# Amos-Chen98/neo-planner

Hardware: AMD Instinct MI355X
Metric: trajectories/sec (batched replan) (higher is better)
Workload: dtype f32x; 1 GPU; cfg2: 40 x 4096 trajectories x 20 waypoints per step per GPU, 1 x 300^3 f32 ESDF per GPU (trilinear, pillars + 80 canopy boxes), each optimised to L-BFGS-B termination; batch_per_launch=4096, pieces=21, dims=3, esdf_voxels=27000000, layout=brick, parallelism=scene-sharded x1, launches_in_flight_per_gpu=4

## Files before the change

neo-planner_amd/csrc/neo_device.hpp:

```cpp
#pragma once
#include <type_traits>
#include <hip/hip_runtime.h>
#include <hip/hip_fp16.h>

#include "../../include/neo_planner.h"
#include "neo_wave.hpp"

namespace neo {

constexpr int kSlots = 4;

struct DevParams {
  double v_max, T_min, T_max, safe_dis, delta_t;
  double w[4];
  double coll_tol;
  double ftol, gtol;
  int maxls, maxiter, maxfun, stale_T;
  int dbg;
  struct F32 {
    float T_min, T_span;
    float dt, inv_dt;
    float vmax2, safe;
    float w[4];
  } f;
// ... 103 lines not shown
  }
};

template <typename E>
__device__ __forceinline__ float elem_to_float(E v);
template <>
__device__ __forceinline__ float elem_to_float<float>(float v) { return v; }
template <>
__device__ __forceinline__ float elem_to_float<__half>(__half v) { return __half2float(v); }

typedef unsigned long long u64_align4 __attribute__((aligned(4)));
typedef unsigned int u32_align2 __attribute__((aligned(2)));
template <typename E>
__device__ __forceinline__ void load_pair(const E *p, float &a, float &b);
template <>
__device__ __forceinline__ void load_pair<float>(const float *p, float &a, float &b) {
  const unsigned long long u = *reinterpret_cast<const u64_align4 *>(p);
  a = __uint_as_float((unsigned int)(u & 0xffffffffull));
  b = __uint_as_float((unsigned int)(u >> 32));
}
__device__ __forceinline__ void buffer_load_pair_f32(__amdgpu_buffer_rsrc_t rsrc, unsigned int off, unsigned int soff,
                                                     float &a, float &b) {
  const auto v = __builtin_amdgcn_raw_buffer_load_b64(rsrc, (int)off, (int)soff, 0);
  a = __uint_as_float(v[0]);
  b = __uint_as_float(v[1]);
}
template <>
__device__ __forceinline__ void load_pair<__half>(const __half *p, float &a, float &b) {
  const unsigned int u = *reinterpret_cast<const u32_align2 *>(p);
  a = __half2float(__ushort_as_half((unsigned short)(u & 0xffffu)));
  b = __half2float(__ushort_as_half((unsigned short)(u >> 16)));
}

template <typename Real, typename E, int LAYOUT>
struct Lookup3D {
  const Map3D &m;
  __amdgpu_buffer_rsrc_t rsrc;
  float inv, off[3], hi[3];
  __device__ __forceinline__ explicit Lookup3D(const Map3D &m_)
      : m(m_), rsrc(__builtin_amdgcn_make_buffer_rsrc(const_cast<void *>(m_.data), 0, (int)m_.bytes, 0x00020000)) {
    inv = m_.f_inv;
#pragma unroll
    for (int k = 0; k < 3; ++k) {
      off[k] = m_.f_off[k];
      hi[k] = m_.f_hi[k];
    }
  }
  struct Addr {
    int i0[3];
    Real fr[3];
    bool inside;
  };
  struct Raw {
    float c[2][2][2];
  };
  static constexpr bool gather_ahead = sizeof(E) == 4;
  static __device__ __forceinline__ void pin(Raw &q) {
#pragma unroll
    for (int k = 0; k < 8; ++k) q.c[k >> 2][(k >> 1) & 1][k & 1] = opaque(q.c[k >> 2][(k >> 1) & 1][k & 1]);
  }

  template <int D>
  __device__ __forceinline__ Addr prepare(const Real (&pos)[D], bool on = true) const {
#pragma clang fp contract(on)
    static_assert(D == 3, "the 3-D map needs D = 3");
    const int n[3] = {m.nx, m.ny, m.nz};
    const double org[3] = {m.ox, m.oy, m.oz};
    Addr a;
    a.inside = on;
    if constexpr (sizeof(Real) == 4) {
#pragma unroll
      for (int k = 0; k < 3; ++k) {
        const float um = fmaf(pos[k], inv, off[k]);
        if (!(um >= -0.5f && um < hi[k])) a.inside = false;
        const int i = min(max((int)floorf(um), 0), n[k] - 2);
        a.i0[k] = i;
        a.fr[k] = __builtin_amdgcn_fmed3f(um - (float)i, 0.0f, 1.0f);
      }
      if (!a.inside) a.i0[0] = a.i0[1] = a.i0[2] = 0;
      return a;
    }
#pragma unroll
    for (int k = 0; k < 3; ++k) {
      Real u = (Real)(((double)pos[k] - org[k]) * m.d_inv);
      if (!(u >= Real(0) && u < (Real)n[k])) a.inside = false;
      u -= Real(0.5);
      const int i = min(max((int)floor(u), 0), n[k] - 2);
      a.i0[k] = i;
      a.fr[k] = fmin(fmax(u - (Real)i, Real(0)), Real(1));
    }
    if (!a.inside) a.i0[0] = a.i0[1] = a.i0[2] = 0;
    return a;
  }
  __device__ __forceinline__ Raw load(const Addr &a) const {
    const E *vox = static_cast<const E *>(m.data);
    Raw q;
    if (LAYOUT == 2 || (LAYOUT == 9 && m.layout == NEO_LAYOUT_CELL8)) {
      const unsigned int cell = __umul24(__umul24((unsigned)a.i0[2], (unsigned)m.ny) + (unsigned)a.i0[1], (unsigned)m.nx) +
                                (unsigned)a.i0[0];
      if constexpr (sizeof(E) == 4) {
        const auto lo = __builtin_amdgcn_raw_buffer_load_b128(rsrc, (int)(cell * 32u), 0, 0);
        const auto hi = __builtin_amdgcn_raw_buffer_load_b128(rsrc, (int)(cell * 32u + 16u), 0, 0);
        q.c[0][0][0] = __uint_as_float(lo[0]); q.c[0][0][1] = __uint_as_float(lo[1]);
        q.c[0][1][0] = __uint_as_float(lo[2]); q.c[0][1][1] = __uint_as_float(lo[3]);
        q.c[1][0][0] = __uint_as_float(hi[0]); q.c[1][0][1] = __uint_as_float(hi[1]);
        q.c[1][1][0] = __uint_as_float(hi[2]); q.c[1][1][1] = __uint_as_float(hi[3]);
      } else {
        const auto v = __builtin_amdgcn_raw_buffer_load_b128(rsrc, (int)(cell * 16u), 0, 0);
#pragma unroll
        for (int w = 0; w < 4; ++w) {
          q.c[w >> 1][w & 1][0] = __half2float(__ushort_as_half((unsigned short)(v[w] & 0xffffu)));
          q.c[w >> 1][w & 1][1] = __half2float(__ushort_as_half((unsigned short)(v[w] >> 16)));
        }
      }
    } else if (LAYOUT == 3 || (LAYOUT == 9 && m.layout == NEO_LAYOUT_BRICK)) {
      constexpr int SHX = sizeof(E) == 4 ? 1 : 2, CX = (1 << SHX) + 1;
      const unsigned int bx = (unsigned)a.i0[0] >> SHX, by = (unsigned)a.i0[1] >> 1, bz = (unsigned)a.i0[2] >> 1;
      const unsigned int lx = (unsigned)a.i0[0] & ((1u << SHX) - 1u), ly = (unsigned)a.i0[1] & 1u, lz = (unsigned)a.i0[2] & 1u;
      const unsigned int blk = __umul24(__umul24(bz, (unsigned)m.nby) + by, (unsigned)m.nbx) + bx;
      const unsigned int in_line = (lz * 3u + ly) * (unsigned)CX + lx;
#pragma unroll
      for (int dz = 0; dz < 2; ++dz)
#pragma unroll
        for (int dy = 0; dy < 2; ++dy) {
          const unsigned int so = (unsigned)((dz * 3 + dy) * CX);
          if constexpr (sizeof(E) == 4) {
            const auto v = __builtin_amdgcn_raw_buffer_load_b64(rsrc, (int)(blk * 128u + in_line * 4u + so * 4u), 0, 0);
            q.c[dz][dy][0] = __uint_as_float(v[0]);
            q.c[dz][dy][1] = __uint_as_float(v[1]);
          } else {
            load_pair<E>(vox + blk * 64u + in_line + so, q.c[dz][dy][0], q.c[dz][dy][1]);
          }
        }
    } else if (LAYOUT == 0 || (LAYOUT == 9 && m.layout == NEO_LAYOUT_LINEAR)) {
      const unsigned int base = __umul24(__umul24((unsigned)a.i0[2], (unsigned)m.ny) + (unsigned)a.i0[1], (unsigned)m.nx) +
                                (unsigned)a.i0[0];
      const unsigned int sy = (unsigned)m.nx, sz = (unsigned)m.nx * (unsigned)m.ny;
#pragma unroll
      for (int dz = 0; dz < 2; ++dz)
#pragma unroll
        for (int dy = 0; dy < 2; ++dy) {
          const unsigned int so = (dy ? sy : 0u) + (dz ? sz : 0u);
          if constexpr (sizeof(E) == 4)
            buffer_load_pair_f32(rsrc, base * 4u, so * 4u, q.c[dz][dy][0], q.c[dz][dy][1]);
          else
            load_pair<E>(vox + base + so, q.c[dz][dy][0], q.c[dz][dy][1]);
        }
    } else {
      const unsigned int cell = __umul24(__umul24((unsigned)a.i0[2], (unsigned)m.ny) + (unsigned)a.i0[1], (unsigned)m.nx) +
                                (unsigned)a.i0[0];
      if constexpr (sizeof(E) == 4) {
        const auto lo = __builtin_amdgcn_raw_buffer_load_b128(rsrc, (int)(cell * 16u), 0, 0);
        const auto hi = __builtin_amdgcn_raw_buffer_load_b128(rsrc, (int)(cell * 16u + 16u), 0, 0);
        q.c[0][0][0] = __uint_as_float(lo[0]); q.c[0][1][0] = __uint_as_float(lo[1]);
        q.c[1][0][0] = __uint_as_float(lo[2]); q.c[1][1][0] = __uint_as_float(lo[3]);
        q.c[0][0][1] = __uint_as_float(hi[0]); q.c[0][1][1] = __uint_as_float(hi[1]);
        q.c[1][0][1] = __uint_as_float(hi[2]); q.c[1][1][1] = __uint_as_float(hi[3]);
      } else {
        const auto v = __builtin_amdgcn_raw_buffer_load_b128(rsrc, (int)(cell * 8u), 0, 0);
#pragma unroll
        for (int dx = 0; dx < 2; ++dx)
#pragma unroll
          for (int dz = 0; dz < 2; ++dz) {
            const unsigned int u = v[2 * dx + dz];
            q.c[dz][0][dx] = __half2float(__ushort_as_half((unsigned short)(u & 0xffffu)));
            q.c[dz][1][dx] = __half2float(__ushort_as_half((unsigned short)(u >> 16)));
          }
      }
    }
    return q;
  }
  template <int D>
  __device__ __forceinline__ Real finish(const Addr &a, const Raw &q, Real (&g)[D]) const {
#pragma clang fp contract(on)
#pragma unroll
    for (int d = 0; d < D; ++d) g[d] = Real(0);
    if (!a.inside) return Real(10000);
    const Real fx = a.fr[0], fy = a.fr[1], fz = a.fr[2];
    const Real inv_res = sizeof(Real) == 4 ? (Real)m.f_inv : (Real)m.d_inv;
    const Real c000 = (Real)q.c[0][0][0], c100 = (Real)q.c[0][0][1], c010 = (Real)q.c[0][1][0], c110 = (Real)q.c[0][1][1];
    const Real c001 = (Real)q.c[1][0][0], c101 = (Real)q.c[1][0][1], c011 = (Real)q.c[1][1][0], c111 = (Real)q.c[1][1][1];
    const Real dx00 = c100 - c000, dx10 = c110 - c010, dx01 = c101 - c001, dx11 = c111 - c011;
    const Real c00 = c000 + fx * dx00, c10 = c010 + fx * dx10;
    const Real c01 = c001 + fx * dx01, c11 = c011 + fx * dx11;
    const Real c0 = c00 + fy * (c10 - c00), c1 = c01 + fy * (c11 - c01);
    const Real dx0 = dx00 + fy * (dx10 - dx00), dx1 = dx01 + fy * (dx11 - dx01);
    const Real dy0 = c10 - c00, dy1 = c11 - c01;
    g[0] = (dx0 + fz * (dx1 - dx0)) * inv_res;
    g[1] = (dy0 + fz * (dy1 - dy0)) * inv_res;
    g[2] = (c1 - c0) * inv_res;
    return c0 + fz * (c1 - c0);
  }
  template <int D>
  __device__ __forceinline__ Real fetch(const Real (&pos)[D], Real (&g)[D], bool &inside) const {
    const Addr a = prepare<D>(pos);
    inside = a.inside;
    return finish<D>(a, load(a), g);
  }
};

__host__ __device__ __forceinline__ int sample_lanes_per_piece_fwd(int M);

struct WaveLanes {
  static constexpr int W = kWave;
  static constexpr int S = 1;
  static constexpr int dl(int D) { return D; }
  static __device__ __forceinline__ int lane() { return lane_id(); }
  static __device__ __forceinline__ int piece() { return lane_id(); }
  static __device__ __forceinline__ int dim0() { return 0; }
  static __device__ __forceinline__ int base() { return 0; }
  template <class T> static __device__ __forceinline__ T sum_dims(T v) { return v; }
  template <class T> static __device__ __forceinline__ T read(T v, int src ) { return rdlane(v, src); }
  template <class T> static __device__ __forceinline__ T prev(T v, T fill) { return from_prev(v, fill); }
  template <class T> static __device__ __forceinline__ T next(T v, T fill) { return from_next(v, fill); }
  template <class T> static __device__ __forceinline__ T sum(T v) { return wave_sum(v); }
  static __device__ __forceinline__ int any(int pred) { return __any(pred); }
  static __host__ __device__ __forceinline__ int lanes_per_piece(int M);
};

template <int W_>
struct GroupLanes {
  static_assert(W_ == 16 || W_ == 8, "a group is a DPP row or half of one");
  static constexpr int W = W_;
  static constexpr int S = 1;
  static constexpr int dl(int D) { return D; }
  static __device__ __forceinline__ int piece() { return lane_id() & (W - 1); }
  static __device__ __forceinline__ int dim0() { return 0; }
  static __device__ __forceinline__ int lane() { return lane_id() & (W - 1); }
  static __device__ __forceinline__ int base() { return lane_id() & ~(W - 1); }
  template <class T> static __device__ __forceinline__ T sum_dims(T v) { return v; }
  template <class T, class Op>
  static __device__ __forceinline__ T reduce(T v, Op op) {
    if constexpr (W == 16) {
      return __shfl(row_scan(v, op), base() + W - 1, kWave);
    } else {
      v = op(v, dpp<0xB1>(v)); v = op(v, dpp<0x4E>(v)); v = op(v, dpp<0x141>(v));
      return v;
    }
  }
  template <class T> static __device__ __forceinline__ T sum(T v) { return reduce(v, OpAdd()); }
  template <class T> static __device__ __forceinline__ T max_nonneg(T v) { return reduce(v, OpMax()); }
  static __device__ __forceinline__ int any(int pred) {
    return reduce(pred ? 1 : 0, [](int a, int b) { return a | b; });
  }
  template <class T>
  static __device__ __forceinline__ T read(T v, int src ) {
    return __shfl(v, base() + src, kWave);
  }
  template <class T> static __device__ __forceinline__ T prev(T v, T fill) {
    const T o = dpp<0x138>(v);
    return lane() == 0 ? fill : o;
  }
  template <class T> static __device__ __forceinline__ T next(T v, T fill) {
    const T o = dpp<0x130>(v);
    return lane() == W - 1 ? fill : o;
  }
  static __host__ __device__ __forceinline__ int lanes_per_piece(int M) {
    int L = W / M;
    if (L < 1) L = 1;
    if (L >= 8) L = (L >= 16 && W >= 16) ? 16 : 8;
    return L;
  }
};

template <int D_>
struct WaveLanesPD {
  static constexpr int W = kWave;
  static constexpr int S = D_;
  static constexpr int dl(int) { return 1; }
  static __device__ __forceinline__ int lane() { return lane_id(); }
  static __device__ __forceinline__ int base() { return 0; }
  static __device__ __forceinline__ int piece() { return (lane_id() * ((65536 + S - 1) / S)) >> 16; }
  static __device__ __forceinline__ int dim0() { return lane_id() - S * piece(); }
  template <class T> static __device__ __forceinline__ T read(T v, int q ) { return rdlane(v, S * q); }
  template <class T> static __device__ __forceinline__ T prev(T v, T fill) {
#pragma unroll
    for (int k = 0; k < S; ++k) v = dpp<0x138>(v);
    return lane_lt(S) ? fill : v;
  }
  template <class T> static __device__ __forceinline__ T next(T v, T fill) {
#pragma unroll
    for (int k = 0; k < S; ++k) v = dpp<0x130>(v);
    return lane_ge(kWave - S) ? fill : v;
  }
  template <class T> static __device__ __forceinline__ T sum(T v) { return wave_sum(v); }
  static __device__ __forceinline__ int any(int pred) { return __any(pred); }
  template <class T> static __device__ __forceinline__ T sum_dims(T v) {
    T acc = v, t = v;
#pragma unroll
    for (int k = 1; k < S; ++k) {
      t = dpp<0x130>(t);
      acc += t;
    }
    return acc;
  }
  static __host__ __device__ __forceinline__ int lanes_per_piece(int M) { return sample_lanes_per_piece_fwd(M); }
};

struct PlanDynamic {
  static constexpr bool dynamic = true;
  static constexpr bool fold_acc = false, fold_rows = false, pcr_mult = false, pcr_xch = false, sl_cache = false,
                        trace = false, coeff_out = false;
  static constexpr bool gather_ahead = false;
};
struct PlanFixedX {
  static constexpr bool dynamic = false;
  static constexpr bool fold_acc = true, fold_rows = true, pcr_mult = true, pcr_xch = true, sl_cache = true,
                        trace = false, coeff_out = false;
  static constexpr bool gather_ahead = true;
};
template <class Plan, bool K>
__host__ __device__ __forceinline__ constexpr bool plan_pick(bool run_time) {
  if constexpr (Plan::dynamic)
    return run_time;
  else
    return K;
}

template <int D, int DL = D, typename Num = double>
struct Traj {
  int M, n, nq, L;
  Num T, tau;
  Num i1, i2, i3, i4;
  Num P0[DL], P1[DL];
  Num V0[DL], A0[DL], V1[DL], A1[DL];
  Num c[6][DL];
  int ns;
  Num N[2][2];
  const double *head, *tail;
  const Num *bnd;
  Num *pcr_xch = nullptr;
  Num *pcr_mult = nullptr;
};

template <int D, class LG, bool TAIL, int DL, typename Num>
__device__ __forceinline__ Num bstate(const Traj<D, DL, Num> &t, int k, int dl) {
  if constexpr (LG::S == 1 && LG::W == kWave)
    return (Num)(TAIL ? t.tail : t.head)[k * D + dl];
  else
    return t.bnd[((TAIL ? 3 : 0) + k) * D + (LG::S > 1 ? LG::dim0() : dl)];
}
template <int D, class LG, int DL, typename Num>
__device__ __forceinline__ void stage_boundary(Traj<D, DL, Num> &t, Num *lds) {
  if constexpr (LG::S > 1) {
    const int lane = lane_id();
    if (lane < 3 * D) lds[lane] = (Num)t.head[lane];
    if (lane < 3 * D) lds[3 * D + lane] = (Num)t.tail[lane];
    lds_wave_sync();
    t.bnd = lds;
  }
}

template <class LG = WaveLanes, typename Num = double>
__device__ __forceinline__ void thomas_factor(int M, const Num (&Lo)[2][2], const Num (&Di)[2][2],
                                              const Num (&Up)[2][2], Num (&N)[2][2], Num (&E)[2][2]) {
  const int lane = LG::piece();
#pragma unroll
  for (int i = 0; i < 2; ++i)
#pragma unroll
    for (int j = 0; j < 2; ++j) N[i][j] = E[i][j] = Num(0.0);
  for (int p = 1; p < M; ++p) {
    const Num e00 = LG::read(E[0][0], p - 1), e01 = LG::read(E[0][1], p - 1);
    const Num e10 = LG::read(E[1][0], p - 1), e11 = LG::read(E[1][1], p - 1);
    if (lane == p) {
      const Num h00 = fma(-Lo[0][1], e10, fma(-Lo[0][0], e00, Di[0][0]));
      const Num h01 = fma(-Lo[0][1], e11, fma(-Lo[0][0], e01, Di[0][1]));
      const Num h10 = fma(-Lo[1][1], e10, fma(-Lo[1][0], e00, Di[1][0]));
      const Num h11 = fma(-Lo[1][1], e11, fma(-Lo[1][0], e01, Di[1][1]));
      const Num det = fma(h00, h11, -(h01 * h10));
      const Num r = precise_rcp(det);
      N[0][0] = h11 * r;
      N[0][1] = -h01 * r;
      N[1][0] = -h10 * r;
      N[1][1] = h00 * r;
      E[0][0] = fma(N[0][0], Up[0][0], N[0][1] * Up[1][0]);
      E[0][1] = fma(N[0][0], Up[0][1], N[0][1] * Up[1][1]);
      E[1][0] = fma(N[1][0], Up[0][0], N[1][1] * Up[1][0]);
      E[1][1] = fma(N[1][0], Up[0][1], N[1][1] * Up[1][1]);
    }
  }
}

template <int DL, class LG = WaveLanes, typename Num = double>
__device__ __forceinline__ void thomas_solve(int M, const Num (&Lo)[2][2], const Num (&N)[2][2],
                                             const Num (&E)[2][2], const Num (&R)[2][DL],
                                             const Num (&y0)[2][DL], const Num (&yM)[2][DL],
                                             Num (&y)[2][DL]) {
  const int lane = LG::piece();
  Num A[2][2], b[2][DL];
  {
    const bool in = lane >= 1 && lane < M;
    A[0][0] = in ? -(N[0][0] * Lo[0][0] + N[0][1] * Lo[1][0]) : Num(0.0);
    A[0][1] = in ? -(N[0][0] * Lo[0][1] + N[0][1] * Lo[1][1]) : Num(0.0);
    A[1][0] = in ? -(N[1][0] * Lo[0][0] + N[1][1] * Lo[1][0]) : Num(0.0);
    A[1][1] = in ? -(N[1][0] * Lo[0][1] + N[1][1] * Lo[1][1]) : Num(0.0);
#pragma unroll
    for (int d = 0; d < DL; ++d) {
      const Num r0 = N[0][0] * R[0][d] + N[0][1] * R[1][d];
      const Num r1 = N[1][0] * R[0][d] + N[1][1] * R[1][d];
      b[0][d] = lane == 0 ? y0[0][d] : (in ? r0 : Num(0.0));
      b[1][d] = lane == 0 ? y0[1][d] : (in ? r1 : Num(0.0));
    }
  }
  for (int s = 1; s < M; s <<= 1) {
    Num As[2][2], bs[2][DL];
#pragma unroll
    for (int i = 0; i < 2; ++i) {
#pragma unroll
      for (int j = 0; j < 2; ++j) As[i][j] = __shfl_up(A[i][j], s * LG::S, kWave);
#pragma unroll
      for (int d = 0; d < DL; ++d) bs[i][d] = __shfl_up(b[i][d], s * LG::S, kWave);
    }
    if (lane >= s && lane < M) {
#pragma unroll
      for (int d = 0; d < DL; ++d) {
        const Num n0 = A[0][0] * bs[0][d] + A[0][1] * bs[1][d] + b[0][d];
        const Num n1 = A[1][0] * bs[0][d] + A[1][1] * bs[1][d] + b[1][d];
        b[0][d] = n0;
        b[1][d] = n1;
      }
      const Num a00 = A[0][0] * As[0][0] + A[0][1] * As[1][0], a01 = A[0][0] * As[0][1] + A[0][1] * As[1][1];
      const Num a10 = A[1][0] * As[0][0] + A[1][1] * As[1][0], a11 = A[1][0] * As[0][1] + A[1][1] * As[1][1];
      A[0][0] = a00; A[0][1] = a01; A[1][0] = a10; A[1][1] = a11;
    }
  }
  {
    const bool in = lane >= 1 && lane < M - 1;
#pragma unroll
    for (int d = 0; d < DL; ++d) {
      if (lane == M - 1) {
        b[0][d] -= E[0][0] * yM[0][d] + E[0][1] * yM[1][d];
        b[1][d] -= E[1][0] * yM[0][d] + E[1][1] * yM[1][d];
      }
    }
    A[0][0] = in ? -E[0][0] : Num(0.0);
    A[0][1] = in ? -E[0][1] : Num(0.0);
    A[1][0] = in ? -E[1][0] : Num(0.0);
    A[1][1] = in ? -E[1][1] : Num(0.0);
  }
  for (int s = 1; s < M; s <<= 1) {
    Num As[2][2], bs[2][DL];
#pragma unroll
    for (int i = 0; i < 2; ++i) {
#pragma unroll
      for (int j = 0; j < 2; ++j) As[i][j] = __shfl_down(A[i][j], s * LG::S, kWave);
#pragma unroll
      for (int d = 0; d < DL; ++d) bs[i][d] = __shfl_down(b[i][d], s * LG::S, kWave);
    }
    if (lane >= 1 && lane + s <= M - 1) {
#pragma unroll
      for (int d = 0; d < DL; ++d) {
        const Num n0 = A[0][0] * bs[0][d] + A[0][1] * bs[1][d] + b[0][d];
        const Num n1 = A[1][0] * bs[0][d] + A[1][1] * bs[1][d] + b[1][d];
        b[0][d] = n0;
        b[1][d] = n1;
      }
      const Num a00 = A[0][0] * As[0][0] + A[0][1] * As[1][0], a01 = A[0][0] * As[0][1] + A[0][1] * As[1][1];
      const Num a10 = A[1][0] * As[0][0] + A[1][1] * As[1][0], a11 = A[1][0] * As[0][1] + A[1][1] * As[1][1];
      A[0][0] = a00; A[0][1] = a01; A[1][0] = a10; A[1][1] = a11;
    }
  }
#pragma unroll
  for (int d = 0; d < DL; ++d) {
    y[0][d] = b[0][d];
    y[1][d] = b[1][d];
  }
}

template <int DL, class LG, typename Num, class Plan = PlanDynamic>
__device__ __forceinline__ void pcr_solve(int M, Num (&L)[2][2], Num (&Dg)[2][2], Num (&U)[2][2], Num (&R)[2][DL],
                                          Num (&y)[2][DL], Num *mult = nullptr, Num *xch = nullptr) {
  static_assert(LG::W == kWave, "written for lane groups that span the wavefront");
  const int p = LG::piece();
  const bool in = p >= 1 && p < M;
#pragma unroll
  for (int i = 0; i < 2; ++i) {
#pragma unroll
    for (int j = 0; j < 2; ++j) {
      L[i][j] = in ? L[i][j] : Num(0.0);
      U[i][j] = in ? U[i][j] : Num(0.0);
      Dg[i][j] = in ? Dg[i][j] : Num(i == j ? 1.0 : 0.0);
    }
#pragma unroll
    for (int d = 0; d < DL; ++d) R[i][d] = in ? R[i][d] : Num(0.0);
  }
  const int lane = lane_id();
  const int s_end = sizeof(Num) == 4 ? min(M - 1, 32) : M - 1;
  typedef Num Quad __attribute__((ext_vector_type(4)));
  const bool keep = plan_pick<Plan, Plan::pcr_mult>(mult != nullptr), use_xch = plan_pick<Plan, Plan::pcr_xch>(xch != nullptr);
  const bool writer = keep && in && LG::dim0() == opaque_uniform(0);
  int level = 0;
  if constexpr (sizeof(Num) == 4) {
    typedef float f2 __attribute__((ext_vector_type(2)));
    auto fma2 = [](f2 x, f2 y, f2 z) { return __builtin_elementwise_fma(x, y, z); };
    f2 Lr[2] = {{L[0][0], L[0][1]}, {L[1][0], L[1][1]}}, Dr[2] = {{Dg[0][0], Dg[0][1]}, {Dg[1][0], Dg[1][1]}};
    f2 Ur[2] = {{U[0][0], U[0][1]}, {U[1][0], U[1][1]}}, Ir[2];
    auto invert = [&]() {
      const float det = fmaf(Dr[0].x, Dr[1].y, -(Dr[0].y * Dr[1].x));
      const float r = precise_rcp(det);
      Ir[0].x = Dr[1].y * r;
      Ir[0].y = -Dr[0].y * r;
      Ir[1].x = -Dr[1].x * r;
      Ir[1].y = Dr[0].x * r;
    };
    auto fetch = [&](const f2 v, int src) { return f2{__shfl(v.x, src, kWave), __shfl(v.y, src, kWave)}; };
    const int ps = min(p, M);
    for (int s = 1; s < s_end; s <<= 1, ++level) {
      invert();
      const int sp = lane - s * LG::S, sn = lane + s * LG::S;
      f2 Ip[2], Lp[2], Upv[2], In[2], Ln[2], Un[2];
      Num Rp[2][DL], Rn[2][DL];
      if (use_xch) {
        Quad *tab = reinterpret_cast<Quad *>(xch);
        f2 *rx = reinterpret_cast<f2 *>(xch + (size_t)(M + 1) * 12);
        lds_wave_sync();
        tab[ps * 3 + 0] = Quad{Ir[0].x, Ir[0].y, Ir[1].x, Ir[1].y};
        tab[ps * 3 + 1] = Quad{Lr[0].x, Lr[0].y, Lr[1].x, Lr[1].y};
        tab[ps * 3 + 2] = Quad{Ur[0].x, Ur[0].y, Ur[1].x, Ur[1].y};
#pragma unroll
        for (int d = 0; d < DL; ++d) rx[lane * DL + d] = f2{R[0][d], R[1][d]};
        lds_wave_sync();
        const int pp = min(max(p - s, 0), M - 1), pn = min(p + s, M - 1);
        const Quad qi = tab[pp * 3 + 0], ql = tab[pp * 3 + 1], qu = tab[pp * 3 + 2];
        const Quad ni = tab[pn * 3 + 0], nl = tab[pn * 3 + 1], nu = tab[pn * 3 + 2];
        Ip[0] = qi.xy; Ip[1] = qi.zw; Lp[0] = ql.xy; Lp[1] = ql.zw; Upv[0] = qu.xy; Upv[1] = qu.zw;
        In[0] = ni.xy; In[1] = ni.zw; Ln[0] = nl.xy; Ln[1] = nl.zw; Un[0] = nu.xy; Un[1] = nu.zw;
#pragma unroll
        for (int d = 0; d < DL; ++d) {
          const f2 rp = rx[(sp & (kWave - 1)) * DL + d], rn = rx[(sn & (kWave - 1)) * DL + d];
          Rp[0][d] = rp.x; Rp[1][d] = rp.y;
          Rn[0][d] = rn.x; Rn[1][d] = rn.y;
        }
      } else {
#pragma unroll
        for (int i = 0; i < 2; ++i) {
          Ip[i] = fetch(Ir[i], sp);
          Upv[i] = fetch(Ur[i], sp);
          In[i] = fetch(Ir[i], sn);
          Ln[i] = fetch(Lr[i], sn);
          Lp[i] = fetch(Lr[i], sp);
          Un[i] = fetch(Ur[i], sn);
#pragma unroll
          for (int d = 0; d < DL; ++d) {
            Rp[i][d] = __shfl(R[i][d], sp, kWave);
            Rn[i][d] = __shfl(R[i][d], sn, kWave);
          }
        }
      }
      f2 pa[2], pg[2];
#pragma unroll
      for (int i = 0; i < 2; ++i) {
        pa[i] = fma2(Lr[i].xx, Ip[0], Lr[i].yy * Ip[1]);
        pg[i] = fma2(Ur[i].xx, In[0], Ur[i].yy * In[1]);
      }
      if (keep) {
        Quad *dst = reinterpret_cast<Quad *>(mult + ((size_t)level * (M + 1) + ps) * 8);
        dst[0] = Quad{pa[0].x, pa[0].y, pa[1].x, pa[1].y};
        dst[1] = Quad{pg[0].x, pg[0].y, pg[1].x, pg[1].y};
      }
#pragma unroll
      for (int i = 0; i < 2; ++i) {
        const f2 ai = -pa[i], gi = -pg[i];
        const f2 ln2 = fma2(ai.xx, Lp[0], ai.yy * Lp[1]);
        const f2 un2 = fma2(gi.xx, Un[0], gi.yy * Un[1]);
        Dr[i] = fma2(gi.yy, Ln[1], fma2(gi.xx, Ln[0], fma2(ai.yy, Upv[1], fma2(ai.xx, Upv[0], Dr[i]))));
#pragma unroll
        for (int d = 0; d < DL; ++d)
          R[i][d] = fmaf(gi.y, Rn[1][d], fmaf(gi.x, Rn[0][d], fmaf(ai.y, Rp[1][d], fmaf(ai.x, Rp[0][d], R[i][d]))));
        Lr[i] = ln2;
        Ur[i] = un2;
      }
    }
    invert();
    if (use_xch) lds_wave_sync();
    if (keep) *reinterpret_cast<Quad *>(mult + (size_t)level * (M + 1) * 8 + (size_t)ps * 4) = Quad{Ir[0].x, Ir[0].y, Ir[1].x, Ir[1].y};
#pragma unroll
    for (int d = 0; d < DL; ++d) {
      y[0][d] = fmaf(Ir[0].x, R[0][d], Ir[0].y * R[1][d]);
      y[1][d] = fmaf(Ir[1].x, R[0][d], Ir[1].y * R[1][d]);
    }
    return;
  }
  Num I[2][2];
  auto invert = [&]() {
    const Num det = fma(Dg[0][0], Dg[1][1], -(Dg[0][1] * Dg[1][0]));
    const Num r = precise_rcp(det);
    I[0][0] = Dg[1][1] * r;
    I[0][1] = -Dg[0][1] * r;
    I[1][0] = -Dg[1][0] * r;
    I[1][1] = Dg[0][0] * r;
  };
  for (int s = 1; s < s_end; s <<= 1, ++level) {
    invert();
    const int lp = lane - s * LG::S, ln = lane + s * LG::S;
    const int sp = lp >= 0 ? lp : lane, sn = ln < kWave ? ln : lane;
    const bool last = 2 * s >= s_end;
    Num Ip[2][2], Lp[2][2], Upv[2][2], Rp[2][DL], In[2][2], Ln[2][2], Un[2][2], Rn[2][DL];
#pragma unroll
    for (int i = 0; i < 2; ++i) {
#pragma unroll
      for (int j = 0; j < 2; ++j) {
        Ip[i][j] = __shfl(I[i][j], sp, kWave);
        Upv[i][j] = __shfl(U[i][j], sp, kWave);
        In[i][j] = __shfl(I[i][j], sn, kWave);
        Ln[i][j] = __shfl(L[i][j], sn, kWave);
        Lp[i][j] = Un[i][j] = Num(0.0);
        if (!last) {
          Lp[i][j] = __shfl(L[i][j], sp, kWave);
          Un[i][j] = __shfl(U[i][j], sn, kWave);
        }
      }
#pragma unroll
// ... 950 lines not shown
```

neo-planner_amd/csrc/neo_kernels.hpp:

```cpp
#pragma once
#include <type_traits>
#include <hip/hip_runtime.h>
#include <hip/hip_fp16.h>

#include "../../include/neo_planner.h"
#ifndef NEO_FUSED_U
#define NEO_FUSED_U (sizeof(Real) == 4 ? 4 : 2)
#endif
#ifndef NEO_W2_U
#define NEO_W2_U 1
#endif
#ifndef NEO_W2_OCC
#define NEO_W2_OCC 2
#endif
#ifndef NEO_X_OCC
#define NEO_X_OCC 3
#endif
#ifndef NEO_SM_MAX_SLOTS
#define NEO_SM_MAX_SLOTS 2
#endif
#ifndef NEO_W2_MAX_SLOTS
#define NEO_W2_MAX_SLOTS 4
#endif
#include "neo_device.hpp"
#include "neo_lbfgs.hpp"
#include "neo_lbfgs_sm.hpp"

namespace neo {

template <typename Num, int NS>
using opt_scalar_t = std::conditional_t<sizeof(Num) == 4 && (NS <= NEO_SM_MAX_SLOTS), float, double>;

template <int D, int NS, typename Real>
__host__ __device__ constexpr int stage_doubles() {
  constexpr int fold = sizeof(Real) == 4 ? kWave * 8 * D * (int)sizeof(Real) : 0;
  return (NS * kWave * 8 > fold ? NS * kWave * 8 : fold) / 8;
}

constexpr int kSlCacheInts = kWave / 4 + kWave + 4;

template <typename Real, int NS, int WAVES>
__host__ __device__ constexpr bool pairs_in_f32() {
  return sizeof(Real) == 4 && WAVES == 2 && NS > 2;
}
template <int D, int NS, typename Real, class MapT, class LookupT, int SU = NEO_FUSED_U, class LG = WaveLanes,
          bool PAIRS32 = false, typename Num = double, class Plan = PlanDynamic>
struct DevBackend {
  static constexpr int DL = LG::dl(D);
  static constexpr int kSlotsN = NS;
  static constexpr bool kPcr = sizeof(Num) == 4 && LG::W == kWave;
  static constexpr bool kAhead = !Plan::dynamic && Plan::gather_ahead && LookupT::gather_ahead && SU == 1 && sizeof(Real) == 4;
  struct Vec {
    Num v[NS];
  };
  Traj<D, DL, Num> t;
  const DevParams &prm;
  const MapT &map;
  double *xs;
  static constexpr int kStage = stage_doubles<D, NS, Real>();
  int *sl_cache = nullptr;
  bool fold_rows = true;
  bool fold_acc = false;
  using Scalar = opt_scalar_t<Num, NS>;
  LineSearchT<Scalar> *lsp;
  double *cst;
  using Hist = std::conditional_t<PAIRS32, float, double>;
  Hist *hist;
  int npad, m;
  double *coeff_out;
  long long samples = 0;
  int last_ns = 0;
  double *trace = nullptr;
  double *trace_xg = nullptr;
  int trace_cap = 0;

  __device__ DevBackend(const DevParams &p, const MapT &mp) : prm(p), map(mp) {}

  __device__ __forceinline__ double dot(const Vec &a, const Vec &b) const {
    Num s = Num(0);
#pragma unroll
    for (int k = 0; k < NS; ++k) s += a.v[k] * b.v[k];
    return uni((double)wave_sum(s));
  }
  __device__ __forceinline__ double uni(double v) const { return uniform(v); }
  __device__ __forceinline__ float uni(float v) const { return uniform(v); }
  __device__ __forceinline__ double amax(const Vec &a) const {
    Num s = Num(0);
#pragma unroll
    for (int k = 0; k < NS; ++k) s = fmax(s, fabs(a.v[k]));
    return wave_max_nonneg(s);
  }
  __device__ __forceinline__ void copy(Vec &d, const Vec &s) const {
#pragma unroll
    for (int k = 0; k < NS; ++k) d.v[k] = s.v[k];
  }
  __device__ __forceinline__ void neg(Vec &d, const Vec &s) const {
#pragma unroll
    for (int k = 0; k < NS; ++k) d.v[k] = -s.v[k];
  }
  __device__ __forceinline__ void axpy(double a, const Vec &x, Vec &y) const {
#pragma unroll
    for (int k = 0; k < NS; ++k) y.v[k] += (Num)a * x.v[k];
  }
  __device__ __forceinline__ void lincomb(Vec &o, const Vec &a, double s, const Vec &b) const {
#pragma unroll
    for (int k = 0; k < NS; ++k) o.v[k] = a.v[k] + (Num)s * b.v[k];
  }
  __device__ __forceinline__ void scale(Vec &v, double s) const {
#pragma unroll
    for (int k = 0; k < NS; ++k) v.v[k] *= (Num)s;
  }
  static constexpr int kFull = NS == 3 ? 2 : NS / 2;
  __device__ __forceinline__ bool in_range(int k, int lane) const { return k < kFull || k * kWave + lane < t.n; }
  __device__ __forceinline__ void hist_put(int slot, const Vec &s, const Vec &y) {
    const int lane = lane_id();
#pragma unroll
    for (int k = 0; k < NS; ++k)
      if (in_range(k, lane)) {
        hist[slot * t.n + k * kWave + lane] = (Hist)s.v[k];
        hist[(m + slot) * t.n + k * kWave + lane] = (Hist)y.v[k];
      }
    lds_wave_sync();
  }
  __device__ __forceinline__ void hist_get(int row, Vec &v) const {
    const int lane = lane_id();
#pragma unroll
    for (int k = 0; k < NS; ++k) v.v[k] = in_range(k, lane) ? (Num)hist[row * t.n + k * kWave + lane] : Num(0);
  }
  __device__ __forceinline__ void hist_get_s(int slot, Vec &v) const { hist_get(slot, v); }
  __device__ __forceinline__ void hist_get_y(int slot, Vec &v) const { hist_get(m + slot, v); }
  __device__ __forceinline__ void hist_get_sy(int slot, Vec &s, Vec &y) const {
    const int lane = lane_id();
    const Hist *ps = hist + slot * t.n + lane, *py = hist + (m + slot) * t.n + lane;
#pragma unroll
    for (int k = 0; k < NS; ++k) {
      s.v[k] = Num(0);
      y.v[k] = Num(0);
      if (in_range(k, lane)) {
        s.v[k] = (Num)ps[k * kWave];
        y.v[k] = (Num)py[k * kWave];
      }
    }
  }
  Num sreg = Num(0);
  __device__ __forceinline__ void sput(int i, double v) { sreg = (lane_id() == i) ? (Num)v : sreg; }
  __device__ __forceinline__ double sget(int i) const { return (double)rdlane(sreg, i); }
  __device__ __forceinline__ double sdiff(int i, double b) const { return (double)(rdlane(sreg, i) - (Num)b); }
  __device__ __forceinline__ double rho_dot(int slot, const Vec &a, const Vec &b) const {
    Num s = Num(0);
#pragma unroll
    for (int k = 0; k < NS; ++k) s += a.v[k] * b.v[k];
    return (double)(rdlane(sreg, slot) * wave_sum(s));
  }
  static constexpr bool kOwnDirection = sizeof(Num) == 4;
  __device__ __forceinline__ void direction(const Vec &g, Vec &d, int col, int head, int mm, Num theta) {
    if (col == 0) {
      neg(d, g);
      return;
    }
    auto slot_of = [&](int k) { return head + k < mm ? head + k : head + k - mm; };
    auto dot3 = [&](const Vec &a0, const Vec &b0, const Vec &a1, const Vec &b1, const Vec &a2, const Vec &b2, Num &t0, Num &t1,
                    Num &t2) {
      Num p0 = Num(0), p1 = Num(0), p2 = Num(0);
#pragma unroll
      for (int k = 0; k < NS; ++k) {
        p0 += a0.v[k] * b0.v[k];
        p1 += a1.v[k] * b1.v[k];
        p2 += a2.v[k] * b2.v[k];
      }
      Num unused;
      wave_sum4((float)p0, (float)p1, (float)p2, 0.0f, t0, t1, t2, unused);
    };
    copy(d, g);
    Vec sA, yA, sB, yB;
    int k = col - 1;
    for (; k >= 1; k -= 2) {
      const int A = slot_of(k), B = slot_of(k - 1);
      hist_get_sy(A, sA, yA);
      hist_get_sy(B, sB, yB);
      Num t0, t1, t2;
      dot3(sA, d, sB, d, sB, yA, t0, t1, t2);
      const Num aA = rdlane(sreg, A) * t0;
      const Num aB = rdlane(sreg, B) * (t1 - aA * t2);
      sput(mm + A, (double)aA);
      sput(mm + B, (double)aB);
#pragma unroll
      for (int q = 0; q < NS; ++q) d.v[q] = (d.v[q] - aA * yA.v[q]) - aB * yB.v[q];
    }
    if (k == 0) {
      const int A = slot_of(0);
      hist_get_sy(A, sA, yA);
      const Num aA = (Num)rho_dot(A, sA, d);
      sput(mm + A, (double)aA);
      axpy(-(double)aA, yA, d);
    }
    scale(d, (double)(Num(1) / theta));
    k = 0;
    for (; k + 1 < col; k += 2) {
      const int A = slot_of(k), B = slot_of(k + 1);
      hist_get_sy(A, sA, yA);
      hist_get_sy(B, sB, yB);
      Num t0, t1, t2;
      dot3(yA, d, yB, d, yB, sA, t0, t1, t2);
      const Num cA = rdlane(sreg, mm + A) - rdlane(sreg, A) * t0;
      const Num cB = rdlane(sreg, mm + B) - rdlane(sreg, B) * (t1 + cA * t2);
#pragma unroll
      for (int q = 0; q < NS; ++q) d.v[q] = (d.v[q] + cA * sA.v[q]) + cB * sB.v[q];
    }
    if (k < col) {
      const int A = slot_of(k);
      hist_get_sy(A, sA, yA);
      const double b = rho_dot(A, yA, d);
      axpy(sdiff(mm + A, b), sA, d);
    }
    scale(d, -1.0);
  }

  __device__ __forceinline__ LineSearchT<Scalar> &ls() { return *lsp; }
  __device__ __forceinline__ double *cost_store() { return cst; }

  __device__ __forceinline__ void note_eval(int nfev, int iter, double stp, double f, const Vec &x, const Vec &g) {
    if constexpr (!Plan::dynamic && !Plan::trace) return;
    if (nfev > trace_cap) return;
    if (trace != nullptr && lane_id() == 0) {
      double *r = trace + (size_t)(nfev - 1) * 4;
      r[0] = f;
      r[1] = stp;
      r[2] = (double)last_ns;
      r[3] = (double)iter;
    }
    if (trace_xg != nullptr) {
      const int lane = lane_id();
      double *r = trace_xg + (size_t)(nfev - 1) * 2 * t.n;
#pragma unroll
      for (int k = 0; k < NS; ++k)
        if (k * kWave + lane < t.n) {
          r[k * kWave + lane] = (double)x.v[k];
          r[t.n + k * kWave + lane] = (double)g.v[k];
        }
    }
  }

  __device__ __forceinline__ void scatter_x(const Vec &x) {
    const int lane = opaque(lane_id());
    lds_wave_sync();
    Num *xn = reinterpret_cast<Num *>(xs);
#pragma unroll
    for (int k = 0; k < NS; ++k)
      if (in_range(k, lane)) xn[k * kWave + lane] = x.v[k];
    lds_wave_sync();
    const int M = t.M;
    const int p = opaque(LG::piece());
    const bool act = p < M;
    t.tau = act ? xn[t.nq + p] : Num(0);
#pragma unroll
    for (int d = 0; d < DL; ++d) {
      const int dg = LG::dim0() + d;
      t.P0[d] = (p == 0 || !act) ? bstate<D, LG, false>(t, 0, d) : xn[dg * (M - 1) + (p > 0 ? p - 1 : 0)];
      t.P1[d] = (p >= M - 1) ? bstate<D, LG, true>(t, 0, d) : xn[dg * (M - 1) + p];
    }
  }

  __device__ __forceinline__ int eval(const Vec &x, double &f, Vec &g, double *costs) {
    const int lane = lane_id();
    const int p = LG::piece();
    NEO_MARK("eval_begin");
    const int M_all = t.M;
    t.M = opaque_uniform(M_all);
    scatter_x(x);
    NEO_MARK("scatter_done");
    Num *xn = reinterpret_cast<Num *>(xs);
    double energy, tsum;
    const int st = minco_forward<D, LG, Num, kPcr, Plan>(t, prm, energy, tsum);
    NEO_MARK("forward_done");
    if (st != 0) {
      f = 0.0;
#pragma unroll
      for (int k = 0; k < 4; ++k) costs[k] = 0.0;
      return st;
    }
    if (plan_pick<Plan, Plan::coeff_out>(coeff_out != nullptr) && p < t.M) {
#pragma unroll
      for (int k = 0; k < 6; ++k)
#pragma unroll
        for (int d = 0; d < DL; ++d) coeff_out[(size_t)(6 * p + k) * D + LG::dim0() + d] = (double)t.c[k][d];
    }
    Num gC[6][DL], gT = Num(0);
    double cf, ck;
    {
      Real cr[6][DL], gCr[6][DL], gTr;
#pragma unroll
      for (int k = 0; k < 6; ++k)
#pragma unroll
        for (int d = 0; d < DL; ++d) cr[k][d] = (Real)t.c[k][d];
      LookupT lk(map);
      int ns_by_piece = t.ns;
      if constexpr (LG::S > 1) ns_by_piece = __shfl(t.ns, min(LG::S * lane, kWave - 1), kWave);
      NEO_MARK("assign_begin");
      t.M = opaque_uniform(M_all);
      SampleLanes sl;
      bool cached = false;
      const int ns_key = lane < t.M ? ns_by_piece : 0;
      const bool have_cache = plan_pick<Plan, Plan::sl_cache>(sl_cache != nullptr);
      if (have_cache) cached = __ballot(ns_key == (int)reinterpret_cast<const unsigned char *>(sl_cache)[lane]) == ~0ull;
      if (cached) {
        const unsigned pk = (unsigned)sl_cache[kWave / 4 + lane];
        sl.piece = pk & 63;
        sl.r = (pk >> 6) & 63;
        sl.L = (pk >> 12) & 127;
        sl.act = ((pk >> 19) & 1) != 0;
        sl.first = (pk >> 20) & 63;
        sl.Lp = pk >> 26;
        sl.rounds = __builtin_amdgcn_readfirstlane(sl_cache[kWave / 4 + kWave]);
        sl.lmax = __builtin_amdgcn_readfirstlane(sl_cache[kWave / 4 + kWave + 1]);
        sl.total = __builtin_amdgcn_readfirstlane(sl_cache[kWave / 4 + kWave + 2]);
      } else {
        sl = balanced_sample_lanes<kAhead>(t.M, ns_by_piece, reinterpret_cast<int *>(xs));
        if (have_cache) {
          const bool fits = sl.lmax < 64 && ns_key < 255;
          reinterpret_cast<unsigned char *>(sl_cache)[lane] = (unsigned char)(__ballot(!fits) == 0 ? ns_key : 255);
          sl_cache[kWave / 4 + lane] = (int)((unsigned)sl.piece | ((unsigned)sl.r << 6) | ((unsigned)sl.L << 12) |
                                             ((sl.act ? 1u : 0u) << 19) | ((unsigned)sl.first << 20) | ((unsigned)sl.Lp << 26));
          if (lane == 0) {
            sl_cache[kWave / 4 + kWave] = sl.rounds;
            sl_cache[kWave / 4 + kWave + 1] = sl.lmax;
            sl_cache[kWave / 4 + kWave + 2] = sl.total;
          }
          lds_wave_sync();
        }
      }
      last_ns = sl.total;
      samples += (long long)last_ns;
      NEO_MARK("assign_done");
      minco_sample<Real, D, LookupT, SU, false, LG, Plan>(
          t.M, sl, t.ns, cr, prm, lk, gCr, gTr, cf, ck,
          plan_pick<Plan, Plan::fold_rows>(fold_rows) ? reinterpret_cast<Real *>(xs) : nullptr, fold_acc);
#pragma unroll
      for (int k = 0; k < 6; ++k)
#pragma unroll
        for (int d = 0; d < DL; ++d) gC[k][d] = (Num)gCr[k][d];
      gT = (Num)gTr;
    }
    costs[0] = uniform(energy);
    costs[1] = uniform(tsum);
    costs[2] = uniform(cf);
    costs[3] = uniform(ck);
    f = uniform(costs[0] * prm.w[0] + costs[1] * prm.w[1] + costs[2] * prm.w[2] + costs[3] * prm.w[3]);
    Num gq[DL], gtau;
    NEO_MARK("sample_done");
    t.M = opaque_uniform(M_all);
    if constexpr (kAhead && sizeof(Num) == 4) {
      const Num i1 = opaque(t.i1);
      t.i2 = i1 * i1;
      t.i3 = t.i2 * i1;
      t.i4 = t.i2 * t.i2;
    }
    const int bst = minco_backward<D, LG, Num, kPcr, Plan>(t, prm, gC, gT, gq, gtau);
    NEO_MARK("backward_done");
    if (bst != 0) return bst;
    lds_wave_sync();
    const int pg = opaque(p), lg = opaque(lane);
    if (pg >= 1 && pg < t.M) {
#pragma unroll
      for (int d = 0; d < DL; ++d) xn[(LG::dim0() + d) * (t.M - 1) + pg - 1] = gq[d];
    }
    if (pg < t.M && LG::dim0() == opaque_uniform(0)) xn[t.nq + pg] = gtau;
    lds_wave_sync();
#pragma unroll
    for (int k = 0; k < NS; ++k) g.v[k] = in_range(k, lg) ? xn[k * kWave + lg] : Num(0);
    NEO_MARK("gather_done");
    return 0;
  }
};

__host__ __device__ inline size_t opt_state_doubles(int n, int m) { return 64 + 5 * (size_t)n + kWave + 2 * (size_t)m * (size_t)n; }

template <class BE, class Mach>
__device__ __forceinline__ void save_run(BE &be, const Mach &mc, double *st) {
  const int lane = lane_id(), n = be.t.n;
  lds_wave_sync();
  if (lane == 0) {
    const int iv[9] = {mc.phase, mc.status, mc.nfev, mc.nit, mc.iter, mc.col, mc.head, mc.task, mc.ifun};
#pragma unroll
    for (int k = 0; k < 9; ++k) st[k] = (double)iv[k];
    const double dv[7] = {(double)mc.f, (double)mc.fold, (double)mc.stp, (double)mc.gd, (double)mc.gdold, (double)mc.theta,
                          (double)mc.stp_evaluated};
#pragma unroll
    for (int k = 0; k < 7; ++k) st[9 + k] = dv[k];
    st[16] = (double)be.samples;
    st[17] = (double)be.last_ns;
    const auto &L = *be.lsp;
    const double lv[20] = {(double)L.ftol, (double)L.gtol, (double)L.xtol, (double)L.stpmin, (double)L.stpmax, (double)L.brackt,
                           (double)L.stage, (double)L.ginit, (double)L.gtest, (double)L.gx, (double)L.gy, (double)L.finit,
                           (double)L.fx, (double)L.fy, (double)L.stx, (double)L.sty, (double)L.stmin, (double)L.stmax,
                           (double)L.width, (double)L.width1};
#pragma unroll
    for (int k = 0; k < 20; ++k) st[20 + k] = lv[k];
#pragma unroll
    for (int k = 0; k < 12; ++k) st[40 + k] = be.cst[k];
  }
  double *v = st + 64;
#pragma unroll
  for (int k = 0; k < BE::kSlotsN; ++k)
    if (k * kWave + lane < n) {
      const int e = k * kWave + lane;
      v[e] = (double)mc.x.v[k];
      v[n + e] = (double)mc.g.v[k];
      v[2 * n + e] = (double)mc.t.v[k];
      v[3 * n + e] = (double)mc.r.v[k];
      v[4 * n + e] = (double)mc.d.v[k];
    }
  v[5 * n + lane] = (double)be.sreg;
  double *h = v + 5 * n + kWave;
  for (int i = lane; i < 2 * be.m * n; i += kWave) h[i] = (double)be.hist[i];
}

template <class BE, class Mach>
__device__ __forceinline__ void load_run(BE &be, Mach &mc, const double *st) {
  using Num = decltype(be.sreg);
  const int lane = lane_id(), n = be.t.n;
  auto iu = [&](int k) { return (int)uniform(st[k]); };
  mc.phase = iu(0); mc.status = iu(1); mc.nfev = iu(2); mc.nit = iu(3); mc.iter = iu(4);
  mc.col = iu(5); mc.head = iu(6); mc.task = iu(7); mc.ifun = iu(8);
  using S = typename Mach::S;
  mc.f = (S)uniform(st[9]); mc.fold = (S)uniform(st[10]); mc.stp = (S)uniform(st[11]); mc.gd = (S)uniform(st[12]);
  mc.gdold = (S)uniform(st[13]); mc.theta = (S)uniform(st[14]); mc.stp_evaluated = (S)uniform(st[15]);
  be.samples = (long long)uniform(st[16]);
  be.last_ns = iu(17);
  if (lane == 0) {
    auto &L = *be.lsp;
    L.ftol = (S)st[20]; L.gtol = (S)st[21]; L.xtol = (S)st[22]; L.stpmin = (S)st[23]; L.stpmax = (S)st[24];
    L.brackt = (int)st[25]; L.stage = (int)st[26];
    L.ginit = (S)st[27]; L.gtest = (S)st[28]; L.gx = (S)st[29]; L.gy = (S)st[30]; L.finit = (S)st[31]; L.fx = (S)st[32];
    L.fy = (S)st[33]; L.stx = (S)st[34]; L.sty = (S)st[35]; L.stmin = (S)st[36]; L.stmax = (S)st[37]; L.width = (S)st[38];
    L.width1 = (S)st[39];
#pragma unroll
    for (int k = 0; k < 12; ++k) be.cst[k] = st[40 + k];
  }
  const double *v = st + 64;
#pragma unroll
  for (int k = 0; k < BE::kSlotsN; ++k) {
    const int e = k * kWave + lane;
    const bool in = e < n;
    mc.x.v[k] = in ? (Num)v[e] : Num(0);
    mc.g.v[k] = in ? (Num)v[n + e] : Num(0);
    mc.t.v[k] = in ? (Num)v[2 * n + e] : Num(0);
    mc.r.v[k] = in ? (Num)v[3 * n + e] : Num(0);
    mc.d.v[k] = in ? (Num)v[4 * n + e] : Num(0);
  }
  be.sreg = (Num)v[5 * n + lane];
  const double *h = v + 5 * n + kWave;
  for (int i = lane; i < 2 * be.m * n; i += kWave) be.hist[i] = (typename BE::Hist)h[i];
  lds_wave_sync();
}

template <class LG = WaveLanes, int D, int DL, typename Num>
__device__ __forceinline__ void load_boundary(Traj<D, DL, Num> &t, const double *head, const double *tail, int M,
                                              Num *bnd_lds = nullptr) {
  t.M = M;
  t.nq = D * (M - 1);
  t.n = t.nq + M;
  t.L = sample_lanes_per_piece(M);
  t.head = head;
  t.tail = tail;
  stage_boundary<D, LG>(t, bnd_lds);
}

struct MapTable {
  const void *maps;
};

template <int D, int NS, typename Real, class MapT, class LookupT, class LG = WaveLanes, typename Num = double>
__global__ __launch_bounds__(kWave) void eval_kernel(int B, int M, DevParams prm, MapT map,
                                                      const double *__restrict__ x,
                                                      const double *__restrict__ head,
                                                      const double *__restrict__ tail,
                                                      double *__restrict__ cost, double *__restrict__ costs4,
                                                      double *__restrict__ grad, double *__restrict__ coeffs,
                                                      int *__restrict__ status) {
  __shared__ __attribute__((aligned(16))) double xs[stage_doubles<D, NS, Real>()];
  __shared__ LineSearchT<opt_scalar_t<Num, NS>> lsm;
  __shared__ double cst[12];
  __shared__ Num bnd[6 * D];
  constexpr bool kKeep = sizeof(Num) == 4 && LG::S > 1;
  __shared__ __attribute__((aligned(16))) Num mult_s[kKeep ? (5 * 8 + 4) * (kWave / LG::S + 1) : 4];
  const int b = blockIdx.x;
  if (b >= B) return;
  using BE = DevBackend<D, NS, Real, MapT, LookupT, NEO_FUSED_U, LG, false, Num>;
  BE be(prm, map);
  if constexpr (kKeep) be.t.pcr_mult = mult_s;
  be.xs = xs;
  if constexpr (sizeof(Num) == 4 && LG::W == kWave)
    if (pcr_xch_elems(M, LG::dl(D)) * (int)sizeof(Num) <= stage_doubles<D, NS, Real>() * 8) be.t.pcr_xch = reinterpret_cast<Num *>(xs);
  be.lsp = &lsm;
  be.cst = cst;
  be.hist = nullptr;
  be.m = NEO_LBFGS_M;
  load_boundary<LG>(be.t, head + (size_t)b * 3 * D, tail + (size_t)b * 3 * D, M, bnd);
  const int n = be.t.n;
  be.npad = NS * kWave;
  be.coeff_out = coeffs ? coeffs + (size_t)b * 6 * M * D : nullptr;
  const int lane = lane_id();
  typename BE::Vec xv, gv;
#pragma unroll
  for (int k = 0; k < NS; ++k) xv.v[k] = (k * kWave + lane < n) ? x[(size_t)b * n + k * kWave + lane] : 0.0;
  double f;
  double *costs = cst;
  const int st = be.eval(xv, f, gv, costs);
#pragma unroll
  for (int k = 0; k < NS; ++k)
    if (k * kWave + lane < n) grad[(size_t)b * n + k * kWave + lane] = gv.v[k];
  if (lane == 0) {
    cost[b] = f;
#pragma unroll
    for (int k = 0; k < 4; ++k) costs4[(size_t)b * 4 + k] = costs[k];
    if (status) status[b] = st;
  }
// ... 263 lines not shown
```

neo-planner_amd/csrc/neo_lbfgs_dir.hpp:

```cpp
#pragma once
#include <type_traits>

namespace neo {

template <class Backend, class = void>
struct has_own_direction { static constexpr bool value = false; };
template <class Backend>
struct has_own_direction<Backend, std::enable_if_t<Backend::kOwnDirection>> { static constexpr bool value = true; };

template <class Backend>
NEO_HD void lbfgs_direction(Backend &be, const typename Backend::Vec &g, typename Backend::Vec &d,
                            typename Backend::Vec &tmp, typename Backend::Vec &tmp2, int col, int head, int m,
                            double theta) {
  if constexpr (has_own_direction<Backend>::value) {
    be.direction(g, d, col, head, m, theta);
    return;
  }
  if (col == 0) {
    be.neg(d, g);
    return;
  }
  be.copy(d, g);
  for (int k = col - 1; k >= 0; --k) {
    const int slot = head + k < m ? head + k : head + k - m;
    be.hist_get_sy(slot, tmp, tmp2);
    const double a = be.rho_dot(slot, tmp, d);
    be.sput(m + slot, a);
    be.axpy(-a, tmp2, d);
  }
  be.scale(d, 1.0 / theta);
  for (int k = 0; k < col; ++k) {
    const int slot = head + k < m ? head + k : head + k - m;
    be.hist_get_sy(slot, tmp2, tmp);
    const double b = be.rho_dot(slot, tmp, d);
    be.axpy(be.sdiff(m + slot, b), tmp2, d);
  }
  be.scale(d, -1.0);
}

}
```

Measured before the change: 1.591 million traj/s.

## Add compile-time unrolled full-history L-BFGS direction with prefetched history reads

When the L-BFGS history is full on the fixed-plan path, the two-loop recursion now runs through a compile-time unrolled walker. It keeps every s/y history vector in registers and issues the global loads for the next pair before computing the current pair, so memory latency overlaps with the dot products. In the second loop the vectors are reused from registers instead of being read from memory again. The cost is much higher register pressure (2*M vectors held at once), which could reduce occupancy or cause spills.

Result: faster. 1.681 million traj/s, median of 6 (+5.6%).

```diff
diff --git a/neo-planner_amd/csrc/neo_device.hpp b/neo-planner_amd/csrc/neo_device.hpp
--- a/neo-planner_amd/csrc/neo_device.hpp
+++ b/neo-planner_amd/csrc/neo_device.hpp
@@ -429,12 +429,14 @@
   static constexpr bool fold_acc = false, fold_rows = false, pcr_mult = false, pcr_xch = false, sl_cache = false,
                         trace = false, coeff_out = false;
   static constexpr bool gather_ahead = false;
+  static constexpr bool hist_ahead = false;
 };
 struct PlanFixedX {
   static constexpr bool dynamic = false;
   static constexpr bool fold_acc = true, fold_rows = true, pcr_mult = true, pcr_xch = true, sl_cache = true,
                         trace = false, coeff_out = false;
   static constexpr bool gather_ahead = true;
+  static constexpr bool hist_ahead = true;
 };
 template <class Plan, bool K>
 __host__ __device__ __forceinline__ constexpr bool plan_pick(bool run_time) {
diff --git a/neo-planner_amd/csrc/neo_kernels.hpp b/neo-planner_amd/csrc/neo_kernels.hpp
--- a/neo-planner_amd/csrc/neo_kernels.hpp
+++ b/neo-planner_amd/csrc/neo_kernels.hpp
@@ -153,24 +153,30 @@
     return (double)(rdlane(sreg, slot) * wave_sum(s));
   }
   static constexpr bool kOwnDirection = sizeof(Num) == 4;
+  __device__ __forceinline__ void dot3(const Vec &a0, const Vec &b0, const Vec &a1, const Vec &b1, const Vec &a2, const Vec &b2,
+                                       Num &t0, Num &t1, Num &t2) const {
+    Num p0 = Num(0), p1 = Num(0), p2 = Num(0);
+#pragma unroll
+    for (int k = 0; k < NS; ++k) {
+      p0 += a0.v[k] * b0.v[k];
+      p1 += a1.v[k] * b1.v[k];
+      p2 += a2.v[k] * b2.v[k];
+    }
+    Num unused;
+    wave_sum4((float)p0, (float)p1, (float)p2, 0.0f, t0, t1, t2, unused);
+  }
   __device__ __forceinline__ void direction(const Vec &g, Vec &d, int col, int head, int mm, Num theta) {
     if (col == 0) {
       neg(d, g);
       return;
     }
+    if constexpr (!Plan::dynamic && Plan::hist_ahead) {
+      if (col == NEO_LBFGS_M) {
+        direction_full(g, d, head, mm, theta);
+        return;
+      }
+    }
     auto slot_of = [&](int k) { return head + k < mm ? head + k : head + k - mm; };
-    auto dot3 = [&](const Vec &a0, const Vec &b0, const Vec &a1, const Vec &b1, const Vec &a2, const Vec &b2, Num &t0, Num &t1,
-                    Num &t2) {
-      Num p0 = Num(0), p1 = Num(0), p2 = Num(0);
-#pragma unroll
-      for (int k = 0; k < NS; ++k) {
-        p0 += a0.v[k] * b0.v[k];
-        p1 += a1.v[k] * b1.v[k];
-        p2 += a2.v[k] * b2.v[k];
-      }
-      Num unused;
-      wave_sum4((float)p0, (float)p1, (float)p2, 0.0f, t0, t1, t2, unused);
-    };
     copy(d, g);
     Vec sA, yA, sB, yB;
     int k = col - 1;
@@ -213,6 +219,76 @@
       const double b = rho_dot(A, yA, d);
       axpy(sdiff(mm + A, b), sA, d);
     }
+    scale(d, -1.0);
+  }
+  template <int COL>
+  struct DirFull {
+    DevBackend &be;
+    Vec &d;
+    const Num inv_theta;
+    int off[NS];
+    Vec s[COL], y[COL];
+    Num alpha[COL];
+    __device__ __forceinline__ void settle(Vec &sv, Vec &yv) const {
+#pragma unroll
+      for (int k = kFull; k < NS; ++k)
+        if (lane_ge(be.t.n - k * kWave)) {
+          sv.v[k] = Num(0);
+          yv.v[k] = Num(0);
+        }
+    }
+    template <int K>
+    __device__ __forceinline__ void read(int slot) {
+      const Hist *ps = be.hist + slot * be.t.n, *py = be.hist + (be.m + slot) * be.t.n;
+#pragma unroll
+      for (int k = 0; k < NS; ++k) {
+        s[K].v[k] = (Num)ps[off[k]];
+        y[K].v[k] = (Num)py[off[k]];
+      }
+    }
+    template <int KA, int KB>
+    __device__ __forceinline__ void pair1(int A, int B) {
+      settle(s[KA], y[KA]);
+      settle(s[KB], y[KB]);
+      Num t0, t1, t2;
+      be.dot3(s[KA], d, s[KB], d, s[KB], y[KA], t0, t1, t2);
+      const Num aA = rdlane(be.sreg, A) * t0;
+      const Num aB = rdlane(be.sreg, B) * (t1 - aA * t2);
+      alpha[KA] = aA;
+      alpha[KB] = aB;
+#pragma unroll
+      for (int q = 0; q < NS; ++q) d.v[q] = (d.v[q] - aA * y[KA].v[q]) - aB * y[KB].v[q];
+    }
+    template <int KA, int KB>
+    __device__ __forceinline__ void pair2(int A, int B) {
+      Num t0, t1, t2;
+      be.dot3(y[KA], d, y[KB], d, y[KB], s[KA], t0, t1, t2);
+      const Num cA = alpha[KA] - rdlane(be.sreg, A) * t0;
+      const Num cB = alpha[KB] - rdlane(be.sreg, B) * (t1 + cA * t2);
+#pragma unroll
+      for (int q = 0; q < NS; ++q) d.v[q] = (d.v[q] + cA * s[KA].v[q]) + cB * s[KB].v[q];
+    }
+    template <int K>
+    __device__ __forceinline__ void single1(int A) {
+      settle(s[K], y[K]);
+      const Num aA = (Num)be.rho_dot(A, s[K], d);
+      alpha[K] = aA;
+      be.axpy(-(double)aA, y[K], d);
+    }
+    template <int K>
+    __device__ __forceinline__ void single2(int A) {
+      const double b = be.rho_dot(A, y[K], d);
+      be.axpy((double)(alpha[K] - (Num)b), s[K], d);
+    }
+    __device__ __forceinline__ void seam() { be.scale(d, (double)inv_theta); }
+  };
+  __device__ __forceinline__ void direction_full(const Vec &g, Vec &d, int head, int mm, Num theta) {
+    copy(d, g);
+    DirFull<NEO_LBFGS_M> w{*this, d, Num(1) / theta};
+    const int lane = lane_id();
+#pragma unroll
+    for (int k = 0; k < NS; ++k) w.off[k] = in_range(k, lane) ? k * kWave + lane : 0;
+    hist_walk_full<NEO_LBFGS_M>(head, mm, w);
     scale(d, -1.0);
   }
 
diff --git a/neo-planner_amd/csrc/neo_lbfgs_dir.hpp b/neo-planner_amd/csrc/neo_lbfgs_dir.hpp
--- a/neo-planner_amd/csrc/neo_lbfgs_dir.hpp
+++ b/neo-planner_amd/csrc/neo_lbfgs_dir.hpp
@@ -7,6 +7,40 @@
 struct has_own_direction { static constexpr bool value = false; };
 template <class Backend>
 struct has_own_direction<Backend, std::enable_if_t<Backend::kOwnDirection>> { static constexpr bool value = true; };
+
+NEO_HD int hist_slot(int head, int k, int m) { return head + k < m ? head + k : head + k - m; }
+template <int K, class V>
+NEO_HD void hist_full_read1(int head, int m, V &v) {
+  if constexpr (K >= 0) v.template read<K>(hist_slot(head, K, m));
+  if constexpr (K >= 1) v.template read<K - 1>(hist_slot(head, K - 1, m));
+}
+template <int K, class V>
+NEO_HD void hist_full_loop1(int head, int m, V &v) {
+  if constexpr (K >= 0) hist_full_read1<K - 2>(head, m, v);
+  if constexpr (K >= 1) {
+    v.template pair1<K, K - 1>(hist_slot(head, K, m), hist_slot(head, K - 1, m));
+    hist_full_loop1<K - 2>(head, m, v);
+  } else if constexpr (K == 0) {
+    v.template single1<0>(hist_slot(head, 0, m));
+  }
+}
+template <int COL, int K, class V>
+NEO_HD void hist_full_loop2(int head, int m, V &v) {
+  if constexpr (K + 1 < COL) {
+    v.template pair2<K, K + 1>(hist_slot(head, K, m), hist_slot(head, K + 1, m));
+    hist_full_loop2<COL, K + 2>(head, m, v);
+  } else if constexpr (K < COL) {
+    v.template single2<K>(hist_slot(head, K, m));
+  }
+}
+template <int COL, class V>
+NEO_HD void hist_walk_full(int head, int m, V &v) {
+  static_assert(COL >= 1, "at least one pair");
+  hist_full_read1<COL - 1>(head, m, v);
+  hist_full_loop1<COL - 1>(head, m, v);
+  v.seam();
+  hist_full_loop2<COL, 0>(head, m, v);
+}
 
 template <class Backend>
 NEO_HD void lbfgs_direction(Backend &be, const typename Backend::Vec &g, typename Backend::Vec &d,
```
